# arun-sub/genomicsbench

Measured on AMD Instinct MI355X. Metric: bsw_large_gcups, higher is better.
Workload: dtype int32

## Files before the change

### genomicsbench_amd/csrc/bsw_kernels.hip

```cpp
#include "gbx_internal.h"
#include <atomic>
#include <cstdlib>

namespace gbx {
namespace {

constexpr int NEG = -(1 << 29);
constexpr int BIGJ = 1 << 20;

constexpr int NCLS = 21;
constexpr int CLS_LDS = NCLS - 1;
constexpr int NTB = 32;
constexpr int NBIN = NCLS * NTB;
constexpr int HDR = 1024;
constexpr int REG_SCORE_LIMIT = 1 << 20;

struct BswDev {
    int o_del, e_del, o_ins, e_ins, oe_del, oe_ins, zdrop, end_bonus, w, max_mat;
    uint32_t colword[5];
    int32_t col4[5];
    uint32_t row0[5];
    uint32_t row1[5];
    uint8_t remap[24];
    uint32_t lrow[5];
// ... 534 lines not shown
            "v_lshl_or_b32 %[wn], %[v], 16, %[u]\n"
            : [sa] "=&v"(sa), [ta] "=&v"(ta), [tb] "=&v"(tb), [ma] "=&v"(ma), [mb] "=&v"(mb), [x] "=&v"(x), [ha] "=&v"(ha),
              [hb] "=&v"(hb), [td] "=&v"(td), [ed] "=&v"(ed), [ena] "=&v"(ena), [enb] "=&v"(enb), [fd] "=&v"(fd), [ka] "=&v"(ka),
              [kb] "=&v"(kb), [u] "=&v"(u), [v] "=&v"(v), [wn] "=&v"(wn), [f] "+v"(f), [key] "=v"(kout)
            : [w] "v"(w), [qq] "v"(qq), [rw] "v"(rw), [rwn] "v"(rwn), [left] "v"(left), [kin] "v"(kin), [pa] "v"(pa), [pa1] "v"(pa1), [zero] "v"(zero), [oed] "s"(oe_del),
              [edel] "s"(e_del), [eins] "s"(e_ins)
            : "vcc");
    } else {
        int sa, ta, tb, ma, mb, x, ha, td, ti, ed, ena, enb, fd, ka, kb, u, v;
        asm volatile(
            "v_perm_b32 %[sa], %[rwn], %[rw], %[qq]\n"
            "v_cmp_ne_u32_sdwa vcc, %[w], %[zero] src0_sel:BYTE_1 src1_sel:DWORD\n"
            "v_subrev_u32 %[fd], %[eins], %[f]\n"
            "v_add_u32_sdwa %[ta], sext(%[sa]), %[w] dst_sel:DWORD dst_unused:UNUSED_PAD src0_sel:BYTE_0 src1_sel:BYTE_1\n"
            "v_cndmask_b32 %[ma], 0, %[ta], vcc\n"
            "v_cmp_ne_u32_sdwa vcc, %[w], %[zero] src0_sel:BYTE_3 src1_sel:DWORD\n"
            "v_max_i32_sdwa %[x], %[ma], %[w] dst_sel:DWORD dst_unused:UNUSED_PAD src0_sel:DWORD src1_sel:BYTE_0\n"
            "v_add_u32_sdwa %[tb], sext(%[sa]), %[w] dst_sel:DWORD dst_unused:UNUSED_PAD src0_sel:BYTE_1 src1_sel:BYTE_3\n"
            "v_max_i32 %[ha], %[x], %[f]\n"
            "v_subrev_u32 %[td], %[oed], %[ma]\n"
            "v_subrev_u32 %[ti], %[oei], %[ma]\n"
            "v_cndmask_b32 %[mb], 0, %[tb], vcc\n"
            "v_sub_u32_sdwa %[ed], %[w], %[edel] dst_sel:DWORD dst_unused:UNUSED_PAD src0_sel:BYTE_0 src1_sel:DWORD\n"
            "v_max3_i32 %[f], %[fd], %[ti], 0\n"
            "v_max3_i32 %[ena], %[ed], %[td], 0\n"
            "v_max_i32_sdwa %[x], %[mb], %[w] dst_sel:DWORD dst_unused:UNUSED_PAD src0_sel:DWORD src1_sel:BYTE_2\n"
            "v_lshl_or_b32 %[ka], %[ha], 18, %[pa]\n"
            "v_max_i32 %[hb], %[x], %[f]\n"
            "v_subrev_u32 %[td], %[oed], %[mb]\n"
            "v_subrev_u32 %[ti], %[oei], %[mb]\n"
            "v_subrev_u32 %[fd], %[eins], %[f]\n"
            "v_sub_u32_sdwa %[ed], %[w], %[edel] dst_sel:DWORD dst_unused:UNUSED_PAD src0_sel:BYTE_2 src1_sel:DWORD\n"
            "v_max3_i32 %[f], %[fd], %[ti], 0\n"
            "v_max3_i32 %[enb], %[ed], %[td], 0\n"
            "v_lshl_or_b32 %[kb], %[hb], 18, %[pa1]\n"
            "v_lshl_or_b32 %[u], %[left], 8, %[ena]\n"
            "v_lshl_or_b32 %[v], %[ha], 8, %[enb]\n"
            "v_max3_u32 %[key], %[kin], %[ka], %[kb]\n"
            "v_lshl_or_b32 %[wn], %[v], 16, %[u]\n"
            : [sa] "=&v"(sa), [ta] "=&v"(ta), [tb] "=&v"(tb), [ma] "=&v"(ma), [mb] "=&v"(mb), [x] "=&v"(x), [ha] "=&v"(ha),
              [hb] "=&v"(hb), [td] "=&v"(td), [ti] "=&v"(ti), [ed] "=&v"(ed), [ena] "=&v"(ena), [enb] "=&v"(enb), [fd] "=&v"(fd), [ka] "=&v"(ka),
              [kb] "=&v"(kb), [u] "=&v"(u), [v] "=&v"(v), [wn] "=&v"(wn), [f] "+v"(f), [key] "=v"(kout)
            : [w] "v"(w), [qq] "v"(qq), [rw] "v"(rw), [rwn] "v"(rwn), [left] "v"(left), [kin] "v"(kin), [pa] "v"(pa), [pa1] "v"(pa1), [zero] "v"(zero), [oed] "s"(oe_del),
              [oei] "s"(oe_ins), [edel] "s"(e_del), [eins] "s"(e_ins)
            : "vcc");
    }
    left = hb;
    key = kout;
    return wn;
}

#ifdef GBX_BSW_LANE_STATS
__device__ unsigned long long g_bsw_lane_stats[16][4];
#endif
template <bool SYM, bool COMPACT, bool CODE4 = false, bool PACKED = false>
__global__ void __launch_bounds__(64) bsw_lane_kernel(BswDev prm, BswPairs P, BswWork W, int rlo, int rhi, int cols, int slot)
{
    extern __shared__ uint32_t lcell[];
#ifdef GBX_BSW_LANE_STATS
    __shared__ int st_rowmax[2048];
    for (int k = threadIdx.x; k < 2048; k += 64) st_rowmax[k] = 0;
    unsigned long long st_cells = 0, st_rows = 0, st_wcells = 0, st_wrows = 0;
#endif
#define LCELL(byte_addr) (*(uint32_t *)((char *)lcell + (byte_addr)))
#define LCELL16(byte_addr) (*(uint16_t *)((char *)lcell + (byte_addr)))
#define LQ8(byte_addr) (*((uint8_t *)lcell + (byte_addr)))
    const int lane = threadIdx.x;
    const int first = W.lbase[rlo << 8], count = W.lbase[(rhi + 1) << 8] - first;
    const int nchunks = (count + 63) >> 6;
    const int32_t *order = W.lorder + first;
    const int e_ins = prm.e_ins, e_del = prm.e_del, oe_ins = prm.oe_ins, oe_del = prm.oe_del;
    const int cb = lane * 4;
    constexpr int QROW = CODE4 ? 64 : 128;
    const int qb = (cols >> 1) * 256 + (CODE4 ? lane : (lane & 31) * 4 + (lane >> 5) * 2);
    auto LQREAD = [&](int a) -> uint32_t { return CODE4 ? (uint32_t)LQ8(a) : (uint32_t)LCELL16(a); };
    auto QSEL = [](uint32_t q) -> uint32_t { return CODE4 ? (((q >> 4) << 8) | (q & 15u)) : q; };
    auto QLOW = [](uint32_t q) -> uint32_t { return CODE4 ? (q & 15u) : (q & 0xffu); };
    auto cell_at = [&](int j) { return COMPACT ? (j >> 1) * 256 + cb + (j & 1) * 2 : j * 256 + cb; };
    const int tab = COMPACT ? (cols >> 1) * (256 + QROW) + 512 : (cols + 2) * 256 - 128;
    if (lane < 5) *(uint4 *)((char *)lcell + tab + lane * 16) = make_uint4(prm.row0[lane], prm.row1[lane], prm.lrow[lane], 0u);
#define LTAB(base_code) (*(const uint4 *)((const char *)lcell + tab + min((int)(base_code), 4) * 16))
    int rel0 = 0, rel1 = 2, rel2 = 256, rel3 = 258, rel4 = 512, rel5 = 514, rel6 = 768, rel7 = 770;
    asm volatile("" : "+v"(rel0), "+v"(rel1), "+v"(rel2), "+v"(rel3), "+v"(rel4), "+v"(rel5), "+v"(rel6), "+v"(rel7));
    for (;;) {
        int c = 0;
        if (lane == 0) c = atomicAdd(&W.lchunk[slot], 1);
        c = __builtin_amdgcn_readfirstlane(c);
        if (c >= nchunks) break;
        const int hi_ = count - (c << 6), idx = hi_ - 64 + lane;
        const bool have = idx >= 0;
        const int pair = order[have ? idx : 0];
        const int qlen = P.len2[pair], tlen = P.len1[pair], h0 = P.h0[pair];
        const int64_t qo = P.idq[pair], to = P.idr[pair];
        const uint8_t *q = P.qer + (PACKED ? 0 : qo);
        const uint8_t *t = P.ref + (PACKED ? 0 : to);
        auto qpiece = [&](int j) -> uint4 {
            uint4 r;
            if (!PACKED) { __builtin_memcpy(&r, q + j, 16); return r; }
            const int64_t o = qo + j;
            const uint8_t *b = q + (o >> 1);
            uint64_t v;
            __builtin_memcpy(&v, b, 8);
            if (o & 1) v = (v >> 4) | ((uint64_t)b[8] << 60);
            auto spread = [](unsigned h) -> unsigned { return (h & 0xfu) | ((h & 0xf0u) << 4) | ((h & 0xf00u) << 8) | ((h & 0xf000u) << 12); };
            const unsigned lo = (unsigned)v, hi = (unsigned)(v >> 32);
            r.x = spread(lo & 0xffffu); r.y = spread(lo >> 16); r.z = spread(hi & 0xffffu); r.w = spread(hi >> 16);
            return r;
        };
        auto tbase = [&](int i) -> int {
            if (!PACKED) return t[i];
            const int64_t o = to + i;
            return (t[o >> 1] >> ((int)(o & 1) * 4)) & 15;
        };
        {
            uint4 wq = qpiece(0);
            int hrun = h0 - oe_ins + e_ins;
            for (int j0 = 0; j0 <= qlen; j0 += 16) {
                const uint4 cur = wq;
                if (j0 + 16 <= qlen) wq = qpiece(j0 + 16);
                const uint32_t ww[4] = {cur.x, cur.y, cur.z, cur.w};
#pragma unroll
                for (int c = 0; c < 16; c += 2) {
                    const int j = j0 + c;
                    if (j <= qlen) {
                        const uint32_t two = (ww[c >> 2] >> ((c & 3) * 8)) & 0xffffu;
                        const int c0 = j < qlen ? min((int)(two & 0xffu), 4) : 0, c1 = j + 1 < qlen ? min((int)(two >> 8), 4) : 0;
                        const int hv0 = j == 0 ? h0 : max(hrun, 0), hv1 = max(hrun - e_ins, 0);
                        hrun -= 2 * e_ins;
                        if (COMPACT) {
                            LCELL((j >> 1) * 256 + cb) = ((uint32_t)hv0 << 8) | ((uint32_t)hv1 << 24);
                            if (CODE4) LQ8(qb + (j >> 1) * QROW) = (uint8_t)(c0 | (c1 << 4));
                            else LCELL16(qb + (j >> 1) * QROW) = (uint16_t)(c0 | (c1 << 8));
                        } else {
                            LCELL(cell_at(j)) = ((uint32_t)hv0 << 18) | (uint32_t)(c0 * 6);
                            if (j + 1 <= qlen) LCELL(cell_at(j + 1)) = ((uint32_t)hv1 << 18) | (uint32_t)(c1 * 6);
                        }
                    }
                }
            }
        }
        const int w = band_width(prm, qlen);
        int best = h0, best_i = -1, best_j = -1, g_i = -1, g_score = -1, off = 0;
        int beg = 0, end = qlen;
        uint4 mrow = LTAB(tbase(0)), mnext = LTAB(tbase(1));
        int tb2 = tbase(2);
        const uint8_t *tp = t + 3;
        int hrow = h0 - prm.o_del - e_del;
        int imw = -w, ipw = w + 1;
        for (int i = 0; i < tlen; ++i) {
            const uint32_t rw = COMPACT ? mrow.x : mrow.z, rwn = mrow.y;
            mrow = mnext;
            mnext = LTAB(tb2);
            if (PACKED) tb2 = tbase(i + 3);
            else tb2 = *tp++;
            beg = max(beg, imw);
            end = min(min(end, ipw), qlen);
            ++imw; ++ipw;
#ifdef GBX_BSW_LANE_STATS
            if (have) { st_cells += (unsigned)max(end - beg, 0); st_rows += 1; atomicMax(&st_rowmax[i & 2047], max(end - beg, 0) + 1); }
#endif
            int left = beg == 0 ? max(hrow, 0) : 0;
            hrow -= e_del;
            int f = 0;
            uint32_t key = 0;
            int vzero = 0;
            asm volatile("" : "+v"(vzero));
            uint32_t sb0 = 0, sb1 = 0, se0 = 0, se1 = 0;
            const int sp0 = beg >> 1, sq = max((end >> 1) - 1, 0);
            if (COMPACT) {
                auto step = [&](int diag, int e, uint32_t qc, int at) -> uint32_t {
                    const int sc = (int)(int8_t)__builtin_amdgcn_perm(rwn, rw, qc);
                    const int m = diag ? diag + sc : 0;
                    const int h = imax3(m, e, f);
                    key = max(key, ((uint32_t)h << 18) | (uint32_t)at);
                    const int td = m - oe_del;
                    const int en = imax3(e - e_del, td, 0);
                    f = imax3(f - e_ins, SYM ? td : m - oe_ins, 0);
                    const uint32_t cell = ((uint32_t)left << 8) | (uint32_t)en;
                    left = h;
                    return cell;
                };
                const bool odd_first = (beg & 1) && beg < end;
                int j = odd_first ? beg - 1 : beg;
                int pa = (j >> 1) * 256 + cb, qa = qb + (j >> 1) * QROW;
                uint32_t w0 = LCELL(pa), q0 = LQREAD(qa), w1 = LCELL(pa + 256), q1 = LQREAD(qa + QROW);
                w0 &= odd_first ? 0xffff0000u : 0xffffffffu;
                for (; j + 7 < end; j += 8, pa += 1024, qa += 4 * QROW) {
                    const uint32_t x0 = LCELL(pa + 512), y0 = LQREAD(qa + 2 * QROW), x1 = LCELL(pa + 768), y1 = LQREAD(qa + 3 * QROW);
                    uint32_t kt;
                    LCELL(pa) = lane_pair_step<SYM>(w0, QSEL(q0), rw, rwn, f, left, (uint32_t)vzero, kt, rel0, rel1, vzero, oe_del, oe_ins, e_del, e_ins);
                    LCELL(pa + 256) = lane_pair_step<SYM>(w1, QSEL(q1), rw, rwn, f, left, kt, kt, rel2, rel3, vzero, oe_del, oe_ins, e_del, e_ins);
                    w0 = LCELL(pa + 1024); q0 = LQREAD(qa + 4 * QROW); w1 = LCELL(pa + 1280); q1 = LQREAD(qa + 5 * QROW);
                    LCELL(pa + 512) = lane_pair_step<SYM>(x0, QSEL(y0), rw, rwn, f, left, kt, kt, rel4, rel5, vzero, oe_del, oe_ins, e_del, e_ins);
                    LCELL(pa + 768) = lane_pair_step<SYM>(x1, QSEL(y1), rw, rwn, f, left, kt, kt, rel6, rel7, vzero, oe_del, oe_ins, e_del, e_ins);
                    key = max(key, kt + (uint32_t)pa);
                }
                if (j + 3 < end) {
                    const uint32_t x0 = LCELL(pa + 512), y0 = LQREAD(qa + 2 * QROW);
                    LCELL(pa) = lane_pair_step<SYM>(w0, QSEL(q0), rw, rwn, f, left, key, key, pa, pa + 2, vzero, oe_del, oe_ins, e_del, e_ins);
                    LCELL(pa + 256) = lane_pair_step<SYM>(w1, QSEL(q1), rw, rwn, f, left, key, key, pa + 256, pa + 258, vzero, oe_del, oe_ins, e_del, e_ins);
                    w0 = x0; q0 = y0;
                    w1 = LCELL(pa + 768); q1 = LQREAD(qa + 3 * QROW);
                    j += 4; pa += 512; qa += 2 * QROW;
                }
                if (j + 1 < end) {
                    LCELL(pa) = lane_pair_step<SYM>(w0, QSEL(q0), rw, rwn, f, left, key, key, pa, pa + 2, vzero, oe_del, oe_ins, e_del, e_ins);
                    w0 = w1; q0 = q1;
                    j += 2; pa += 256; qa += QROW;
                }
                if (j < end) {
                    LCELL16(pa) = (uint16_t)step((int)((w0 >> 8) & 0xffu), (int)(w0 & 0xffu), QLOW(q0), pa);
                }
                LCELL16(cell_at(end)) = (uint16_t)(left << 8);
                sb0 = LCELL(sp0 * 256 + cb); sb1 = LCELL(sp0 * 256 + 256 + cb);
                se0 = LCELL(sq * 256 + cb); se1 = LCELL(sq * 256 + 256 + cb);
            } else {
                uint32_t left18 = (uint32_t)left << 18;
                int ab = cell_at(beg);
                const int abend = cell_at(end);
                uint32_t cw = LCELL(ab);
#pragma unroll 2
                for (; ab < abend; ab += 256) {
                    const uint32_t nw = LCELL(ab + 256);
                    const int diag = (int)(cw >> 18), e = (int)((cw >> 5) & 0x1fffu);
                    const uint32_t qo = cw & 31u;
                    const int sc = __builtin_amdgcn_sbfe((int)rw, qo, 6u);
                    const int m = diag ? diag + sc : 0;
                    const int h = imax3(m, e, f);
                    const uint32_t h18 = (uint32_t)h << 18;
                    key = max(key, h18 | (uint32_t)ab);
                    const int td = m - oe_del;
                    const int en = imax3(e - e_del, td, 0);
                    f = imax3(f - e_ins, SYM ? td : m - oe_ins, 0);
                    LCELL(ab) = left18 | ((uint32_t)en << 5) | qo;
                    left18 = h18;
                    cw = nw;
                }
                left = (int)(left18 >> 18);
                LCELL(abend) = left18 | (LCELL(abend) & 31u);
            }
            const int jfin = beg < end ? end : beg;
            if (jfin == qlen) {
                if (!(g_score > left)) g_i = i;
                g_score = max(g_score, left);
            }
            const int row_best = (int)(key >> 18);
            const int karg = (int)(key & 0x3ffffu) - cb;
            const int row_arg = COMPACT ? ((karg >> 8) << 1) | ((karg >> 1) & 1) : karg >> 8;
            if (row_best == 0) break;
            if (row_best > best) {
                best = row_best; best_i = i; best_j = row_arg;
                off = max(off, abs(row_arg - i));
            } else if (prm.zdrop > 0) {
                const int di = i - best_i, dj = row_arg - best_j;
                if (di > dj) { if (best - row_best - (di - dj) * e_del > prm.zdrop) break; }
                else if (best - row_best - (dj - di) * e_ins > prm.zdrop) break;
            }
            int j = beg;
            if (COMPACT) {
                int k = (sb1 >> 16) ? 3 : 4;
                k = (sb1 & 0xffffu) ? 2 : k;
                k = (sb0 >> 16) ? 1 : k;
                k = (sb0 & 0xffffu) && !(beg & 1) ? 0 : k;
                j = 2 * sp0 + k;
                if (k == 4) while (j < end && LCELL16(cell_at(j)) == 0) ++j;
                j = min(j, end);
                const int nbeg = beg < end ? j : beg;
                const int khi = end - 2 * sq;
                k = (se0 & 0xffffu) ? 0 : -1;
                k = (se0 >> 16) && khi >= 1 ? 1 : k;
                k = (se1 & 0xffffu) && khi >= 2 ? 2 : k;
                k = (se1 >> 16) && khi >= 3 ? 3 : k;
                j = 2 * sq + k;
                if (k < 0 && 2 * sq > nbeg) while (j >= nbeg && LCELL16(cell_at(j)) == 0) --j;
                j = max(j, nbeg - 1);
                j = nbeg > end ? end : j;
                beg = nbeg;
            } else {
                while (j < end && LCELL(cell_at(j)) < 32u) ++j;
                beg = j;
                j = end;
                while (j >= beg && LCELL(cell_at(j)) < 32u) --j;
            }
            end = min(j + 2, qlen);
        }
        gbx_bsw_result r;
        r.score = best; r.tle = best_i + 1; r.gtle = g_i + 1; r.qle = best_j + 1; r.gscore = g_score; r.max_off = off;
        if (have) P.out[pair] = r;
#ifdef GBX_BSW_LANE_STATS
        __builtin_amdgcn_s_waitcnt(0);
        for (int k = threadIdx.x; k < 2048; k += 64) { const int m = st_rowmax[k]; if (m) { st_wcells += 64ull * (unsigned)(m - 1); st_wrows += 64; } st_rowmax[k] = 0; }
#endif
    }
#ifdef GBX_BSW_LANE_STATS
    atomicAdd(&g_bsw_lane_stats[slot][0], st_cells); atomicAdd(&g_bsw_lane_stats[slot][1], st_wcells);
    atomicAdd(&g_bsw_lane_stats[slot][2], st_rows); atomicAdd(&g_bsw_lane_stats[slot][3], st_wrows);
#endif
#undef LCELL
#undef LCELL16
#undef LQ8
#undef LTAB
}

struct RowShape { int lpp, cpl; };
typedef void (*RowsFn)(BswDev, BswPairs, BswWork, int);
struct RowKernel { int lpp, cpl; RowsFn fn[2]; std::atomic<int> bpc[2]; const char *name; };
#define GBX_ROW_KERNEL(L, C) { L, C, { bsw_rows_kernel<L, C, false>, bsw_rows_kernel<L, C, true> }, { 0, 0 }, "bsw_rows_" #L "x" #C }
RowKernel row_kernels[] = {
    GBX_ROW_KERNEL(2, 4),  GBX_ROW_KERNEL(2, 8),  GBX_ROW_KERNEL(2, 12), GBX_ROW_KERNEL(2, 16), GBX_ROW_KERNEL(2, 20), GBX_ROW_KERNEL(2, 24),
    GBX_ROW_KERNEL(4, 14), GBX_ROW_KERNEL(4, 16), GBX_ROW_KERNEL(4, 18), GBX_ROW_KERNEL(4, 20), GBX_ROW_KERNEL(4, 22), GBX_ROW_KERNEL(4, 24),
    GBX_ROW_KERNEL(8, 13), GBX_ROW_KERNEL(8, 14), GBX_ROW_KERNEL(8, 15), GBX_ROW_KERNEL(8, 16),
    GBX_ROW_KERNEL(16, 10), GBX_ROW_KERNEL(16, 12), GBX_ROW_KERNEL(16, 16), GBX_ROW_KERNEL(64, 16),
    GBX_ROW_KERNEL(4, 8), GBX_ROW_KERNEL(4, 12), GBX_ROW_KERNEL(8, 10), GBX_ROW_KERNEL(8, 12), GBX_ROW_KERNEL(16, 8),
    GBX_ROW_KERNEL(64, 3), GBX_ROW_KERNEL(64, 4),
};
#undef GBX_ROW_KERNEL
constexpr int class_qmax[NCLS - 1] = {8, 16, 24, 32, 40, 48, 56, 64, 72, 80, 88, 96, 104, 112, 120, 128, 160, 192, 256, 1024};

constexpr uint8_t CLASS_REMAP[3][NCLS] = {
    {0, 1, 2, 3, 4, 5, 6, 7, 8, 9, 10, 11, 12, 13, 14, 15, 16, 17, 18, 19, 20},
    {3, 3, 3, 3, 7, 7, 7, 7, 11, 11, 11, 11, 15, 15, 15, 15, 18, 18, 18, 19, 20},
    {15, 15, 15, 15, 15, 15, 15, 15, 15, 15, 15, 15, 15, 15, 15, 15, 18, 18, 18, 19, 20},
};
int class_mode_for(int64_t n)
{
    const char *e = getenv("GBX_BSW_CLASSMODE");
    if (e && *e >= '0' && *e <= '2') return *e - '0';
    return n < 32768 ? 2 : n < 250000 ? 1 : 0;
}

RowKernel *find_row_kernel(int lpp, int cpl)
{
    for (RowKernel &k : row_kernels)
        if (k.lpp == lpp && k.cpl == cpl) return &k;
    return nullptr;
}

const RowShape *class_shapes()
{
    static RowShape shapes[NCLS - 1] = {{2, 4},  {2, 8},  {2, 12}, {2, 16}, {2, 20}, {2, 24}, {4, 14}, {4, 16}, {4, 18}, {4, 20},
                                        {4, 22}, {4, 24}, {8, 13}, {8, 14}, {8, 15}, {8, 16}, {16, 10}, {16, 12}, {16, 16}, {64, 16}};
    static bool parsed = false;
    if (!parsed) {
        parsed = true;
        const char *e = getenv("GBX_BSW_SHAPES");
        for (int c = 0; e && *e && c < NCLS - 1; ++c) {
            int l = 0, k = 0, used = 0;
            if (sscanf(e, "%dx%d%n", &l, &k, &used) != 2) break;
            if (find_row_kernel(l, k) && l * k >= class_qmax[c]) shapes[c] = {l, k};
            e += used;
            if (*e == ',') ++e;
        }
    }
    return shapes;
}

int make_dev_params(const gbx_bsw_params *p, BswDev *d)
{
    if (p->e_del < 1 || p->e_ins < 1 || p->o_del < 0 || p->o_ins < 0 || p->e_del > 4096 || p->e_ins > 4096 ||
        p->o_del > (1 << 16) || p->o_ins > (1 << 16) || p->w < 0) {
        set_error("bsw: gap penalties must satisfy 0<=o<=65536, 1<=e<=4096, w>=0");
        return GBX_ERR_ARG;
    }
    d->o_del = p->o_del; d->e_del = p->e_del; d->o_ins = p->o_ins; d->e_ins = p->e_ins;
    d->oe_del = p->o_del + p->e_del; d->oe_ins = p->o_ins + p->e_ins;
    d->zdrop = p->zdrop; d->end_bonus = p->end_bonus; d->w = p->w;
    int mx = 0;
    for (int k = 0; k < 25; ++k) mx = p->mat[k] > mx ? p->mat[k] : mx;
    d->max_mat = mx;
    for (int q = 0; q < 5; ++q) {
        uint32_t wv = 0;
        for (int t = 0; t < 4; ++t) wv |= (uint32_t)(uint8_t)p->mat[t * 5 + q] << (8 * t);
        d->colword[q] = wv;
        d->col4[q] = p->mat[4 * 5 + q];
    }
    for (int t = 0; t < 5; ++t) {
        uint32_t wv = 0;
        for (int q = 0; q < 4; ++q) wv |= (uint32_t)(uint8_t)p->mat[t * 5 + q] << (8 * q);
        d->row0[t] = wv;
        d->row1[t] = (uint32_t)(uint8_t)p->mat[t * 5 + 4];
    }
    d->lane_on = 0;
    bool fits6 = true;
    for (int k = 0; k < 25; ++k) fits6 = fits6 && p->mat[k] >= -32 && p->mat[k] <= 31;
    for (int t = 0; t < 5; ++t) {
        uint32_t wv = 0;
        for (int q = 0; q < 5; ++q) wv |= ((uint32_t)p->mat[t * 5 + q] & 63u) << (6 * q);
        d->lrow[t] = wv;
    }
    if (fits6 && p->o_del + p->e_del < LANE_SCORE_LIMIT && p->o_ins + p->e_ins < LANE_SCORE_LIMIT) d->lane_on = -1;
    return GBX_OK;
}

}

constexpr int64_t WS_LANE = (int64_t)(LANE_BINS + 64) + 64;
size_t bsw_workspace_bytes(int64_t n)
{
    return (size_t)(WS_HDR + 4 * (n > 0 ? n : 0) + WS_LANE) * sizeof(int32_t);
}

constexpr int UNPACK_ROUNDS = 4;
__global__ void __launch_bounds__(256) bsw_unpack4_kernel(const uint8_t *__restrict__ packed, uint8_t *__restrict__ out, int64_t lo, int64_t hi)
{
    const int64_t base = lo + (int64_t)blockIdx.x * (256 * 16 * UNPACK_ROUNDS) + threadIdx.x * 16;
    const bool aligned = (((uintptr_t)(packed + (base >> 1)) & 7) == 0) && (((uintptr_t)(out + base) & 15) == 0);
    if (aligned && base + (int64_t)(UNPACK_ROUNDS - 1) * 4096 + 16 <= hi) {
        uint2 v[UNPACK_ROUNDS];
#pragma unroll
        for (int r = 0; r < UNPACK_ROUNDS; ++r) v[r] = *(const uint2 *)(packed + ((base + r * 4096) >> 1));
        auto spread = [](unsigned h) -> unsigned { return (h & 0xfu) | ((h & 0xf0u) << 4) | ((h & 0xf00u) << 8) | ((h & 0xf000u) << 12); };
#pragma unroll
        for (int r = 0; r < UNPACK_ROUNDS; ++r) {
            uint4 q;
            q.x = spread(v[r].x & 0xffffu); q.y = spread(v[r].x >> 16); q.z = spread(v[r].y & 0xffffu); q.w = spread(v[r].y >> 16);
            *(uint4 *)(out + base + r * 4096) = q;
        }
        return;
    }
    for (int r = 0; r < UNPACK_ROUNDS; ++r) {
        const int64_t o = base + r * 4096;
        if (o >= hi) return;
        if (aligned && o + 16 <= hi) {
            const uint2 v = *(const uint2 *)(packed + (o >> 1));
            auto spread = [](unsigned h) -> unsigned { return (h & 0xfu) | ((h & 0xf0u) << 4) | ((h & 0xf00u) << 8) | ((h & 0xf000u) << 12); };
            uint4 q;
            q.x = spread(v.x & 0xffffu); q.y = spread(v.x >> 16); q.z = spread(v.y & 0xffffu); q.w = spread(v.y >> 16);
            *(uint4 *)(out + o) = q;
        } else {
            for (int64_t k = o; k < o + 16 && k < hi; ++k) out[k] = (uint8_t)((packed[k >> 1] >> ((k & 1) * 4)) & 0xf);
        }
    }
}

int bsw_unpack4(const uint8_t *d_packed, uint8_t *d_out, int64_t lo, int64_t hi, hipStream_t s)
{
    if (hi <= lo) return GBX_OK;
    const int64_t per_block = 256 * 16 * UNPACK_ROUNDS;
    Stage st("bsw_unpack4", s);
    hipLaunchKernelGGL(bsw_unpack4_kernel, dim3((unsigned)((hi - lo + per_block - 1) / per_block)), dim3(256), 0, s, d_packed, d_out, lo, hi);
    GBX_HIP(hipGetLastError());
    return GBX_OK;
}

int bsw_launch_direct(const gbx_bsw_params *p, int64_t n, int max_qlen,
                      const uint8_t *d_ref, const uint8_t *d_qer, const int64_t *d_idr, const int64_t *d_idq,
                      const int32_t *d_len1, const int32_t *d_len2, const int32_t *d_h0, gbx_bsw_result *d_out, hipStream_t s)
{
    if (n <= 0) return GBX_OK;
    BswDev dev;
    int rc = make_dev_params(p, &dev);
    if (rc) return rc;
    for (int c = 0; c < NCLS; ++c) dev.remap[c] = (uint8_t)c;
    BswPairs P = {d_ref, d_qer, d_idr, d_idq, d_len1, d_len2, d_h0, d_out};
    BswWork W = {nullptr, nullptr, nullptr, nullptr, nullptr, nullptr, nullptr, nullptr, nullptr, nullptr};
    dev.lane_on = 0;
    if (max_qlen > 256) { set_error("bsw: direct launch needs queries of at most 256"); return GBX_ERR_ARG; }
    const int cols = max_qlen + 1;
    int lpp = 16, cpl = cols <= 128 ? 8 : cols <= 160 ? 10 : cols <= 192 ? 12 : 16;
    if (n < 4096) { lpp = 64; cpl = cols <= 192 ? 3 : 4; }
    if (const char *e = getenv("GBX_BSW_DIRECT_SHAPE")) {
        int l = 0, c = 0;
        if (sscanf(e, "%dx%d", &l, &c) == 2 && l * c > max_qlen && find_row_kernel(l, c)) { lpp = l; cpl = c; }
    }
    RowKernel *k = find_row_kernel(lpp, cpl);
    if (!k) { set_error("bsw: no %dx%d row kernel", lpp, cpl); return GBX_ERR_UNSUPPORTED; }
    const bool sym = dev.oe_ins == dev.oe_del;
    const int gpb = 256 / lpp;
    const int blocks = (int)((n + gpb - 1) / gpb);
    Stage st(k->name, s);
    hipLaunchKernelGGL(k->fn[sym], dim3(blocks), dim3(256), 0, s, dev, P, W, -(int)n);
    GBX_HIP(hipGetLastError());
    return GBX_OK;
}

static bool lane_wanted(int64_t n)
{
    const char *lane_env = getenv("GBX_BSW_LANE");
    const int64_t lane_min = getenv("GBX_BSW_LANE_MIN") ? atoll(getenv("GBX_BSW_LANE_MIN")) : 262144;
    return lane_env ? atoi(lane_env) != 0 : n >= lane_min;
}

int bsw_lane_rule(const gbx_bsw_params *p, int64_t n, BswLaneRule *r)
{
    BswDev dev;
    const int rc = make_dev_params(p, &dev);
    if (rc) return rc;
    r->on = dev.lane_on && lane_wanted(n) ? 1 : 0;
    r->max_mat = dev.max_mat > 0 ? dev.max_mat : 0;
    r->qmax = LANE_QMAX;
    r->limit = LANE_SCORE_LIMIT;
    r->compact_limit = LANE_COMPACT_LIMIT;
    static_assert(LANE_NRANGE == 5, "BswLaneRule::range_hi / BswChunkPrep::class_pairs");
    for (int f = 0; f < 2; ++f) for (int k = 0; k < LANE_NRANGE; ++k) r->range_hi[f][k] = LANE_RANGE_HI[f][k];
    return GBX_OK;
}

int bsw_launch(const gbx_bsw_params *p, int64_t n,
               const uint8_t *d_ref, const uint8_t *d_qer,
               const int64_t *d_idr, const int64_t *d_idq,
               const int32_t *d_len1, const int32_t *d_len2, const int32_t *d_h0,
               gbx_bsw_result *d_out, void *d_work, size_t work_bytes, hipStream_t s, hipEvent_t *join_events,
               const BswChunkPrep *prep)
{
    if (n == 0) return GBX_OK;
    if (n > 0x7fffffffLL - 1024) { set_error("bsw: more than 2^31 pairs in one call"); return GBX_ERR_UNSUPPORTED; }
    if (work_bytes < bsw_workspace_bytes(n)) { set_error("bsw: workspace too small"); return GBX_ERR_ARG; }
    BswDev dev;
    int rc = make_dev_params(p, &dev);
    if (rc) return rc;
    const int mode = class_mode_for(n);
    for (int c = 0; c < NCLS; ++c) dev.remap[c] = CLASS_REMAP[mode][c];
    BswPairs P = {d_ref, d_qer, d_idr, d_idq, d_len1, d_len2, d_h0, d_out};
    int32_t *wi = (int32_t *)d_work;
    int32_t *wl = wi + WS_HDR + 4 * n;
    BswWork W = {wi, wi + HDR, wi + 2 * HDR, wi + 3 * HDR, wi + WS_HDR, wi + WS_HDR + n, wl, wi + WS_HDR + 3 * n, wi + WS_HDR + 2 * n,
                 wl + LANE_BINS + 64};
    dev.lane_on = dev.lane_on && lane_wanted(n) ? 1 : 0;
    static const bool serial = getenv("GBX_BSW_SERIAL") != nullptr;
    SideStreams *ss = nullptr;
    std::unique_lock<std::mutex> side_lock;
    if (!serial) {
        if ((rc = side_streams(&ss))) return rc;
        side_lock = std::unique_lock<std::mutex>(ss->mu);
    }
    static const bool prep_off = getenv("GBX_BSW_PREP") && atoi(getenv("GBX_BSW_PREP")) == 0;
    const bool ahead = prep && prep->uploaded && join_events && !serial && !prep_off;
    hipStream_t s_cls = ahead ? ss->pre[0] : s;
    const bool no_rows = dev.lane_on && prep && prep->rows_pairs == 0 && !(getenv("GBX_BSW_SKIP_ROWS") && atoi(getenv("GBX_BSW_SKIP_ROWS")) == 0);
    const bool packed_lanes = no_rows && prep->ref_packed && !(getenv("GBX_BSW_PACKED_LANES") && atoi(getenv("GBX_BSW_PACKED_LANES")) == 0);
    const int phase = prep ? prep->phase : 0;
    if (phase && !(ahead && packed_lanes && prep->ev_pre && prep->ev_aux)) {
        if (phase == 1) return 1;
        set_error("bsw: the kernels of a chunk whose preparing passes were not queued");
        return GBX_ERR_ARG;
    }
    hipEvent_t ev_pre = phase ? prep->ev_pre : ss ? ss->ev_pre : nullptr, ev_aux = phase ? prep->ev_aux : ss ? ss->ev_aux : nullptr;
    const bool sort_aside = dev.lane_on && !serial;
    if (packed_lanes) { P.ref = prep->ref_packed; P.qer = prep->qer_packed; P.packed = 1; }
    if (phase != 2) {
        if (ahead) {
            GBX_HIP(hipStreamWaitEvent(ss->pre[0], prep->uploaded, 0));
            GBX_HIP(hipStreamWaitEvent(ss->pre[1], prep->uploaded, 0));
        }
        if (!packed_lanes && prep && prep->ref_packed) {
            const int64_t from_r = prep->unp_r ? *prep->unp_r : prep->lo_r, from_q = prep->unp_q ? *prep->unp_q : prep->lo_q;
            if ((rc = bsw_unpack4(prep->ref_packed, prep->ref_bytes, from_r, prep->hi_r, s_cls)) ||
                (rc = bsw_unpack4(prep->qer_packed, prep->qer_bytes, from_q, prep->hi_q, s_cls)))
                return rc;
            if (prep->unp_r && prep->hi_r > *prep->unp_r) *prep->unp_r = prep->hi_r;
            if (prep->unp_q && prep->hi_q > *prep->unp_q) *prep->unp_q = prep->hi_q;
        }
        GBX_HIP(hipMemsetAsync(d_work, 0, WS_HDR * sizeof(int32_t), s_cls));
        if (dev.lane_on) {
            hipStream_t so = s;
            if (ahead) {
                so = ss->pre[1];
                GBX_HIP(hipMemsetAsync(wl, 0, (size_t)WS_LANE * sizeof(int32_t), so));
            } else {
                GBX_HIP(hipMemsetAsync(wl, 0, (size_t)WS_LANE * sizeof(int32_t), s));
                if (sort_aside) {
                    if ((rc = ss->fork(s))) return rc;
                    so = ss->side[SideStreams::N - 1];
                }
            }
            Stage st("bsw_lane_sort", so);
            const int sblocks = (int)((n + 255) / 256);
            hipLaunchKernelGGL(bsw_lane_sort_kernel, dim3(sblocks), dim3(256), 0, so, dev, P, n, W, 0);
            hipLaunchKernelGGL(bsw_lane_scan_kernel, dim3(1), dim3(1024), 0, so, W);
            hipLaunchKernelGGL(bsw_lane_sort_kernel, dim3(sblocks), dim3(256), 0, so, dev, P, n, W, 1);
            if (sort_aside) GBX_HIP(hipEventRecord(ev_aux, so));
        }
        const int cblocks = (int)((n + CLS_THREADS - 1) / CLS_THREADS);
        {
            Stage st("bsw_classify", s_cls);
            hipLaunchKernelGGL(bsw_classify_kernel, dim3(cblocks), dim3(CLS_THREADS), 0, s_cls, dev, P, n, W, 0);
            hipLaunchKernelGGL(bsw_scan_kernel, dim3(1), dim3(HDR), 0, s_cls, W);
            hipLaunchKernelGGL(bsw_classify_kernel, dim3(cblocks), dim3(CLS_THREADS), 0, s_cls, dev, P, n, W, 1);
        }
        if (ahead) GBX_HIP(hipEventRecord(ev_pre, s_cls));
        GBX_HIP(hipGetLastError());
        if (phase == 1) return GBX_OK;
    }
    if (ahead) {
        GBX_HIP(hipStreamWaitEvent(s, ev_pre, 0));
        for (int k = 0; k < SideStreams::N; ++k) GBX_HIP(hipStreamWaitEvent(ss->side[k], ev_pre, 0));
        if (phase == 2) {
            GBX_HIP(hipStreamWaitEvent(s, prep->uploaded, 0));
            for (int k = 0; k < SideStreams::N; ++k) GBX_HIP(hipStreamWaitEvent(ss->side[k], prep->uploaded, 0));
        }
    }

    int dev_id = 0, cus = 256;
    (void)hipGetDevice(&dev_id);
    (void)hipDeviceGetAttribute(&cus, hipDeviceAttributeMultiprocessorCount, dev_id);
    auto grid_for = [&](int groups_per_block, int blocks_per_cu) {
        int64_t want = (n + groups_per_block - 1) / groups_per_block;
        int64_t cap = (int64_t)cus * blocks_per_cu;
        return (int)(want < cap ? want : cap);
    };
    const bool sym = dev.oe_ins == dev.oe_del;
    const RowShape *shapes = class_shapes();
    if (!serial && !sort_aside && !ahead && (rc = ss->fork(s))) return rc;
    int launched = 0;
    for (int c = 0; c < NCLS - 1 && !no_rows; ++c) {
        if (CLASS_REMAP[mode][c] != c) continue;
        static const int nk_env = getenv("GBX_BSW_KSTREAMS") ? atoi(getenv("GBX_BSW_KSTREAMS")) : 0;
        const int nk = nk_env > 0 ? nk_env : join_events ? 3 : 4;
        const int lane_k = mode ? launched++ % (nk > 4 ? 4 : nk) : nk >= 4 ? (c & 3) : c % nk;
        hipStream_t sc = serial || sort_aside || lane_k == 0 ? s : ss->side[lane_k - 1];
        RowKernel *k = find_row_kernel(shapes[c].lpp, shapes[c].cpl);
        if (!k) { set_error("bsw: no row kernel for class %d", c); return GBX_ERR_UNSUPPORTED; }
        int bpc = k->bpc[sym].load(std::memory_order_relaxed);
        if (!bpc) {
            int q = 0;
            if (hipOccupancyMaxActiveBlocksPerMultiprocessor(&q, k->fn[sym], 256, 0) != hipSuccess || q < 1) {
                (void)hipGetLastError();
                q = 2;
            }
            bpc = q > 8 ? 8 : q;
            k->bpc[sym].store(bpc, std::memory_order_relaxed);
        }
        Stage st(k->name, sc);
        hipLaunchKernelGGL(k->fn[sym], dim3(grid_for(256 / k->lpp, bpc)), dim3(256), 0, sc, dev, P, W, c);
    }
    if (sort_aside) {
        GBX_HIP(hipStreamWaitEvent(s, ev_aux, 0));
        for (int k = 0; k + (ahead ? 0 : 1) < SideStreams::N; ++k) GBX_HIP(hipStreamWaitEvent(ss->side[k], ev_aux, 0));
    }
    if (dev.lane_on) {
        static const char *names[2][LANE_NRANGE] = {{"bsw_lane_c47", "bsw_lane_c79", "bsw_lane_c99", "bsw_lane_c135", "bsw_lane_c159"},
                                                    {"bsw_lane_w39", "bsw_lane_w79", "bsw_lane_w103", "bsw_lane_w127", "bsw_lane_w159"}};
        for (int fmt = 1; fmt >= 0; --fmt) {
            int nl = 0;
            for (int r = LANE_NRANGE - 1; r >= 0; --r) {
                const int qlo = r ? LANE_RANGE_HI[fmt][r - 1] + 1 : 1, qhi = LANE_RANGE_HI[fmt][r];
                static const bool skip_on = getenv("GBX_BSW_SKIP_EMPTY") && atoi(getenv("GBX_BSW_SKIP_EMPTY")) == 1;
                if (skip_on && prep && prep->class_known && prep->class_pairs[fmt * LANE_NRANGE + r] == 0) continue;
                ++nl;
                const int cols = (qhi + 3) & ~1;
                const char *c4e = getenv("GBX_BSW_CODE4");
                const bool code4 = fmt == 0 && (c4e ? atoi(c4e) != 0 : qhi > 99);
                const size_t lds = fmt ? (size_t)(cols + 2) * 256 : (size_t)(cols / 2) * (code4 ? 320 : 384) + 640;
                int per_cu = (int)((size_t)160 * 1024 / lds);
                if (per_cu > 16) per_cu = 16;
                const int sk = (nl - 1) & 3;
                hipStream_t sc = serial || sk == 0 ? s : ss->side[sk - 1];
                int64_t blocks = (int64_t)cus * per_cu, want = (n + 63) / 64;
                if (blocks > want) blocks = want;
                const int rlo = fmt * (LANE_QMAX + 1) + qlo, rhi = fmt * (LANE_QMAX + 1) + qhi, slot = fmt * LANE_NRANGE + r;
                Stage st(names[fmt][r], sc);
                auto go = [&](auto kern) { hipLaunchKernelGGL(kern, dim3((unsigned)blocks), dim3(64), lds, sc, dev, P, W, rlo, rhi, cols, slot); };
                if (P.packed) {
                    if (fmt == 0 && code4) { if (sym) go(bsw_lane_kernel<true, true, true, true>); else go(bsw_lane_kernel<false, true, true, true>); }
                    else if (fmt == 0) { if (sym) go(bsw_lane_kernel<true, true, false, true>); else go(bsw_lane_kernel<false, true, false, true>); }
                    else { if (sym) go(bsw_lane_kernel<true, false, false, true>); else go(bsw_lane_kernel<false, false, false, true>); }
                } else if (fmt == 0 && code4) {
                    if (sym) go(bsw_lane_kernel<true, true, true>); else go(bsw_lane_kernel<false, true, true>);
                } else if (fmt == 0) {
                    if (sym) go(bsw_lane_kernel<true, true>); else go(bsw_lane_kernel<false, true>);
                } else {
                    if (sym) go(bsw_lane_kernel<true, false>); else go(bsw_lane_kernel<false, false>);
                }
            }
        }
    }
    if (!serial && !join_events && (rc = ss->join(s))) return rc;
    if (!no_rows) {
        const size_t lds_bytes = (size_t)(GBX_BSW_MAX_QLEN + 1) * 2 * sizeof(int);
        static std::atomic<uint64_t> attr_set[2];
        int cur = 0;
        GBX_HIP(hipGetDevice(&cur));
        const uint64_t bit = (uint64_t)1 << (cur & 63);
        if (cur >= 128 || !(attr_set[cur >> 6].load(std::memory_order_acquire) & bit)) {
            GBX_HIP(hipFuncSetAttribute((const void *)bsw_lds_kernel, hipFuncAttributeMaxDynamicSharedMemorySize, (int)lds_bytes));
            if (cur < 128) attr_set[cur >> 6].fetch_or(bit, std::memory_order_release);
        }
        int blocks = (int)(n < (int64_t)cus * 2 ? n : (int64_t)cus * 2);
        Stage st("bsw_lds", s);
        hipLaunchKernelGGL(bsw_lds_kernel, dim3(blocks), dim3(64), lds_bytes, s, dev, P, W, CLS_LDS);
    }
    if (join_events) {
        if (!ss && (rc = side_streams(&ss))) return rc;
        GBX_HIP(hipEventRecord(join_events[0], s));
        for (int k = 0; k < SideStreams::N; ++k) GBX_HIP(hipEventRecord(join_events[1 + k], ss->side[k]));
    }
    GBX_HIP(hipGetLastError());
    return GBX_OK;
}

}

#ifdef GBX_BSW_LANE_STATS
extern "C" int gbx_debug_bsw_lane_stats(unsigned long long *out, int reset)
{
    if (hipMemcpyFromSymbol(out, HIP_SYMBOL(gbx::g_bsw_lane_stats), sizeof(unsigned long long) * 64) != hipSuccess) return -1;
    if (reset) { unsigned long long z[64] = {0}; if (hipMemcpyToSymbol(HIP_SYMBOL(gbx::g_bsw_lane_stats), z, sizeof(z)) != hipSuccess) return -1; }
    return 0;
}
#endif
```

Before: 2435.

## Add register-resident lane kernel with inline-asm cell step for mid-length queries

New measurement: 2524 (median of 6 runs). 3.6% higher.

```diff
diff --git a/genomicsbench_amd/csrc/bsw_kernels.hip b/genomicsbench_amd/csrc/bsw_kernels.hip
--- a/genomicsbench_amd/csrc/bsw_kernels.hip
+++ b/genomicsbench_amd/csrc/bsw_kernels.hip
@@ -860,6 +860,328 @@
 #undef LTAB
 }
 
+
+#define GBX_REG_STEP_HEAD(SEL0, SEL1)                                                                                                   \
+    "v_cmp_ne_u32_sdwa vcc, %[w], %[zero] src0_sel:BYTE_1 src1_sel:DWORD\n"                                                            \
+    "v_subrev_u32 %[fd], %[eins], %[f]\n"                                                                                               \
+    "v_add_u32_sdwa %[ta], sext(%[sa]), %[w] dst_sel:DWORD dst_unused:UNUSED_PAD src0_sel:" SEL0 " src1_sel:BYTE_1\n"                  \
+    "v_cndmask_b32 %[ma], 0, %[ta], vcc\n"                                                                                              \
+    "v_cmp_ne_u32_sdwa vcc, %[w], %[zero] src0_sel:BYTE_3 src1_sel:DWORD\n"                                                            \
+    "v_max_i32_sdwa %[x], %[ma], %[w] dst_sel:DWORD dst_unused:UNUSED_PAD src0_sel:DWORD src1_sel:BYTE_0\n"                            \
+    "v_add_u32_sdwa %[tb], sext(%[sa]), %[w] dst_sel:DWORD dst_unused:UNUSED_PAD src0_sel:" SEL1 " src1_sel:BYTE_3\n"                  \
+    "v_max_i32 %[ha], %[x], %[f]\n"
+#define GBX_REG_STEP_SYM(SEL0, SEL1)                                                                                                    \
+    GBX_REG_STEP_HEAD(SEL0, SEL1)                                                                                                       \
+    "v_subrev_u32 %[td], %[oed], %[ma]\n"                                                                                               \
+    "v_cndmask_b32 %[mb], 0, %[tb], vcc\n"                                                                                              \
+    "v_sub_u32_sdwa %[ed], %[w], %[edel] dst_sel:DWORD dst_unused:UNUSED_PAD src0_sel:BYTE_0 src1_sel:DWORD\n"                         \
+    "v_max3_i32 %[f], %[fd], %[td], 0\n"                                                                                                \
+    "v_max3_i32 %[ena], %[ed], %[td], 0\n"                                                                                              \
+    "v_max_i32_sdwa %[x], %[mb], %[w] dst_sel:DWORD dst_unused:UNUSED_PAD src0_sel:DWORD src1_sel:BYTE_2\n"                            \
+    "v_lshl_or_b32 %[ka], %[ha], 18, %[pa]\n"                                                                                           \
+    "v_max_i32 %[hb], %[x], %[f]\n"                                                                                                     \
+    "v_subrev_u32 %[td], %[oed], %[mb]\n"                                                                                               \
+    "v_subrev_u32 %[fd], %[eins], %[f]\n"                                                                                               \
+    "v_sub_u32_sdwa %[ed], %[w], %[edel] dst_sel:DWORD dst_unused:UNUSED_PAD src0_sel:BYTE_2 src1_sel:DWORD\n"                         \
+    "v_max3_i32 %[f], %[fd], %[td], 0\n"                                                                                                \
+    "v_max3_i32 %[enb], %[ed], %[td], 0\n"                                                                                              \
+    "v_lshl_or_b32 %[kb], %[hb], 18, %[pa1]\n"                                                                                          \
+    "v_lshl_or_b32 %[u], %[left], 8, %[ena]\n"                                                                                          \
+    "v_lshl_or_b32 %[v], %[ha], 8, %[enb]\n"                                                                                            \
+    "v_max3_u32 %[key], %[kin], %[ka], %[kb]\n"                                                                                         \
+    "v_lshl_or_b32 %[wn], %[v], 16, %[u]\n"
+#define GBX_REG_STEP_ASYM(SEL0, SEL1)                                                                                                   \
+    GBX_REG_STEP_HEAD(SEL0, SEL1)                                                                                                       \
+    "v_subrev_u32 %[td], %[oed], %[ma]\n"                                                                                               \
+    "v_subrev_u32 %[ti], %[oei], %[ma]\n"                                                                                               \
+    "v_cndmask_b32 %[mb], 0, %[tb], vcc\n"                                                                                              \
+    "v_sub_u32_sdwa %[ed], %[w], %[edel] dst_sel:DWORD dst_unused:UNUSED_PAD src0_sel:BYTE_0 src1_sel:DWORD\n"                         \
+    "v_max3_i32 %[f], %[fd], %[ti], 0\n"                                                                                                \
+    "v_max3_i32 %[ena], %[ed], %[td], 0\n"                                                                                              \
+    "v_max_i32_sdwa %[x], %[mb], %[w] dst_sel:DWORD dst_unused:UNUSED_PAD src0_sel:DWORD src1_sel:BYTE_2\n"                            \
+    "v_lshl_or_b32 %[ka], %[ha], 18, %[pa]\n"                                                                                           \
+    "v_max_i32 %[hb], %[x], %[f]\n"                                                                                                     \
+    "v_subrev_u32 %[td], %[oed], %[mb]\n"                                                                                               \
+    "v_subrev_u32 %[ti], %[oei], %[mb]\n"                                                                                               \
+    "v_subrev_u32 %[fd], %[eins], %[f]\n"                                                                                               \
+    "v_sub_u32_sdwa %[ed], %[w], %[edel] dst_sel:DWORD dst_unused:UNUSED_PAD src0_sel:BYTE_2 src1_sel:DWORD\n"                         \
+    "v_max3_i32 %[f], %[fd], %[ti], 0\n"                                                                                                \
+    "v_max3_i32 %[enb], %[ed], %[td], 0\n"                                                                                              \
+    "v_lshl_or_b32 %[kb], %[hb], 18, %[pa1]\n"                                                                                          \
+    "v_lshl_or_b32 %[u], %[left], 8, %[ena]\n"                                                                                          \
+    "v_lshl_or_b32 %[v], %[ha], 8, %[enb]\n"                                                                                            \
+    "v_max3_u32 %[key], %[kin], %[ka], %[kb]\n"                                                                                         \
+    "v_lshl_or_b32 %[wn], %[v], 16, %[u]\n"
+template <bool SYM, bool HI, int PA>
+__device__ __forceinline__ uint32_t reg_pair_step(uint32_t w, uint32_t sa, int &f, int &left, uint32_t &key, int zero, int oe_del, int oe_ins,
+                                                  int e_del, int e_ins)
+{
+    uint32_t wn, kout;
+    int hb, ta, tb, ma, mb, x, ha, td, ti, ed, ena, enb, fd, ka, kb, u, v;
+#define GBX_REG_STEP_OPS                                                                                                                \
+    : [ta] "=&v"(ta), [tb] "=&v"(tb), [ma] "=&v"(ma), [mb] "=&v"(mb), [x] "=&v"(x), [ha] "=&v"(ha), [hb] "=&v"(hb), [td] "=&v"(td),   \
+      [ti] "=&v"(ti), [ed] "=&v"(ed), [ena] "=&v"(ena), [enb] "=&v"(enb), [fd] "=&v"(fd), [ka] "=&v"(ka), [kb] "=&v"(kb), [u] "=&v"(u), \
+      [v] "=&v"(v), [wn] "=&v"(wn), [f] "+v"(f), [key] "=v"(kout)                                                                       \
+    : [w] "v"(w), [sa] "v"(sa), [left] "v"(left), [kin] "v"(key), [pa] "i"(PA), [pa1] "i"(PA + 1), [zero] "v"(zero), [oed] "s"(oe_del), \
+      [oei] "s"(oe_ins), [edel] "s"(e_del), [eins] "s"(e_ins)                                                                           \
+    : "vcc"
+    if (SYM && !HI) asm volatile(GBX_REG_STEP_SYM("BYTE_0", "BYTE_1") GBX_REG_STEP_OPS);
+    if (SYM && HI) asm volatile(GBX_REG_STEP_SYM("BYTE_2", "BYTE_3") GBX_REG_STEP_OPS);
+    if (!SYM && !HI) asm volatile(GBX_REG_STEP_ASYM("BYTE_0", "BYTE_1") GBX_REG_STEP_OPS);
+    if (!SYM && HI) asm volatile(GBX_REG_STEP_ASYM("BYTE_2", "BYTE_3") GBX_REG_STEP_OPS);
+#undef GBX_REG_STEP_OPS
+    (void)ti;
+    left = hb;
+    key = kout;
+    return wn;
+}
+#undef GBX_REG_STEP_SYM
+#undef GBX_REG_STEP_ASYM
+#undef GBX_REG_STEP_HEAD
+
+template <bool AND>
+__device__ inline uint32_t wave_bits(uint32_t x)
+{
+    auto op = [](uint32_t a, uint32_t b) { return AND ? a & b : a | b; };
+    int y = (int)x;
+    y = (int)op(y, dpp<0x111>(y, y));
+    y = (int)op(y, dpp<0x112>(y, y));
+    y = (int)op(y, dpp<0x114>(y, y));
+    y = (int)op(y, dpp<0x118>(y, y));
+    y = (int)op(y, dpp<0x142, 0xa>(y, y));
+    y = (int)op(y, dpp<0x143, 0xc>(y, y));
+    return (uint32_t)__builtin_amdgcn_readlane(y, 63);
+}
+__device__ inline uint32_t bits_from(int lo)
+{
+    return lo <= 0 ? ~0u : lo >= 32 ? 0u : ~0u << lo;
+}
+__device__ inline uint32_t bit_span(int lo, int hi)
+{
+    return lo > hi ? 0u : (hi >= 31 ? ~0u : (2u << hi) - 1u) & ~((1u << lo) - 1u);
+}
+
+template <bool SYM, bool HI, int PA>
+__device__ __forceinline__ void reg_pair_masked(uint32_t &cell, uint32_t sa, int beg, int end, int &f, int &left, uint32_t &key,
+                                                int zero, int oe_del, int oe_ins, int e_del, int e_ins)
+{
+    constexpr int c0 = PA;
+    if (c0 + 1 < end && c0 + 1 >= beg) {
+        const uint32_t win = c0 < beg ? cell & 0xffff0000u : cell;
+        cell = reg_pair_step<SYM, HI, PA>(win, sa, f, left, key, zero, oe_del, oe_ins, e_del, e_ins);
+    } else if (c0 + 1 == end) {
+        if (c0 >= beg) {
+            const int sc = (int)(int8_t)(sa >> (HI ? 16 : 0));
+            const int diag = (int)((cell >> 8) & 0xffu), e = (int)(cell & 0xffu);
+            const int m = diag ? diag + sc : 0;
+            const int h = imax3(m, e, f);
+            key = max(key, ((uint32_t)h << 18) | (uint32_t)PA);
+            const int en = imax3(e - e_del, m - oe_del, 0);
+            cell = ((uint32_t)h << 24) | ((uint32_t)left << 8) | (uint32_t)en;
+            left = h;
+        } else {
+            cell = (cell & 0xffffu) | ((uint32_t)left << 24);
+        }
+    } else if (c0 == end) {
+        cell = (cell & 0xffff0000u) | ((uint32_t)left << 8);
+    }
+}
+
+template <bool SYM, int QHI>
+__global__ void __launch_bounds__(64, 3) bsw_lane_reg_kernel(BswDev prm, BswPairs P, BswWork W, int rlo, int rhi, int slot)
+{
+    constexpr int NCP = QHI / 2 + 1;
+    constexpr int NB = (NCP + 3) / 4;
+    constexpr int NQ = (NCP + 1) / 2;
+    constexpr int NW = (2 * NCP + 31) / 32;
+    static_assert(NB <= 31, "block masks are 32-bit");
+    constexpr int OUT = 1 << 12;
+    __shared__ uint2 s_tab[5];
+    const int lane = threadIdx.x;
+    if (lane < 5) s_tab[lane] = make_uint2(prm.row0[lane], prm.row1[lane]);
+    __syncthreads();
+    const int first = W.lbase[rlo << 8], count = W.lbase[(rhi + 1) << 8] - first;
+    const int nchunks = (count + 63) >> 6;
+    const int32_t *order = W.lorder + first;
+    const int e_ins = prm.e_ins, e_del = prm.e_del, oe_ins = prm.oe_ins, oe_del = prm.oe_del;
+    for (;;) {
+        int c = 0;
+        if (lane == 0) c = atomicAdd(&W.lchunk[slot], 1);
+        c = __builtin_amdgcn_readfirstlane(c);
+        if (c >= nchunks) break;
+        const int hi_ = count - (c << 6), idx = hi_ - 64 + lane;
+        const bool have = idx >= 0;
+        const int pair = order[have ? idx : 0];
+        const int qlen = P.len2[pair], tlen = P.len1[pair], h0 = P.h0[pair];
+        const uint8_t *q = P.qer + P.idq[pair];
+        const uint8_t *t = P.ref + P.idr[pair];
+
+        uint32_t qs[NQ];
+#pragma unroll
+        for (int k = 0; k < (4 * NQ + 15) / 16; ++k) {
+            uint4 v = make_uint4(0u, 0u, 0u, 0u);
+            if (16 * k <= qlen) __builtin_memcpy(&v, q + 16 * k, 16);
+            const uint32_t vv[4] = {v.x, v.y, v.z, v.w};
+#pragma unroll
+            for (int m = 0; m < 4 && 4 * k + m < NQ; ++m) {
+                const uint32_t x = vv[m];
+                const uint32_t ge5 = ((((x | 0x80808080u) - 0x05050505u) | x) & 0x80808080u) >> 7;
+                const uint32_t msk = ge5 * 0xffu;
+                qs[4 * k + m] = (x & ~msk) | (0x04040404u & msk);
+            }
+        }
+        uint32_t cell[NCP];
+        {
+            int hr = h0 - oe_ins, rem = qlen;
+#pragma unroll
+            for (int p = 0; p < NCP; ++p) {
+                const int hv0 = p == 0 ? h0 : max(hr + e_ins, 0), hv1 = max(hr, 0);
+                cell[p] = (rem >= 0 ? (uint32_t)hv0 << 8 : 0u) | (rem >= 1 ? (uint32_t)hv1 << 24 : 0u);
+                hr -= 2 * e_ins;
+                rem -= 2;
+            }
+        }
+        const int w = band_width(prm, qlen);
+        int best = h0, best_i = -1, best_j = -1, g_i = -1, g_score = -1, off = 0;
+        int beg = 0, end = qlen;
+        bool running = true;
+        uint2 mrow = s_tab[min((int)t[0], 4)], mnext = s_tab[min((int)t[1], 4)];
+        int tb2 = t[2];
+        const uint8_t *tp = t + 3;
+        int hrow = h0 - prm.o_del - e_del;
+        int imw = -w, ipw = w + 1;
+        for (int i = 0;; ++i) {
+            if (!__any(running)) break;
+            const uint32_t rw = mrow.x, rwn = mrow.y;
+            mrow = mnext;
+            mnext = s_tab[min(tb2, 4)];
+            tb2 = running ? (int)*tp : 0;
+            tp += running ? 1 : 0;
+            beg = max(beg, imw);
+            end = min(min(end, ipw), qlen);
+            ++imw; ++ipw;
+            int left = beg == 0 ? max(hrow, 0) : 0;
+            hrow -= e_del;
+            const int bb = running ? beg : OUT, ee = running ? end : OUT;
+            const int sp0 = bb >> 1, sq = max((ee >> 1) - 1, 0);
+            const uint32_t touch = running ? bit_span(bb >> 3, min(ee >> 3, NB - 1)) : 0u;
+            const uint32_t whole = running ? bit_span((bb + 7) >> 3, min((ee >> 3) - 1, NB - 1)) : ~0u;
+            auto blk = [](int pp) { return pp < 4 * NB ? 1u << (pp >> 2) : 0u; };
+            const uint32_t probe = running ? blk(sp0) | blk(sp0 + 1) | blk(sq) | blk(sq + 1) : 0u;
+            const uint32_t touch_w = wave_bits<false>(touch), whole_w = wave_bits<true>(whole), probe_w = wave_bits<false>(probe);
+            int vzero = 0;
+            asm volatile("" : "+v"(vzero));
+            int f = 0;
+            uint32_t key = 0;
+#pragma unroll
+            for (int b = 0; b < NB; ++b) {
+                if (!((touch_w >> b) & 1u)) continue;
+                const uint32_t sa0 = __builtin_amdgcn_perm(rwn, rw, qs[2 * b]);
+                const uint32_t sa1 = 2 * b + 1 < NQ ? __builtin_amdgcn_perm(rwn, rw, qs[2 * b + 1]) : 0u;
+                uint32_t kt = (uint32_t)vzero;
+                if ((whole_w >> b) & 1u) {
+                    cell[4 * b] = reg_pair_step<SYM, false, 0>(cell[4 * b], sa0, f, left, kt, vzero, oe_del, oe_ins, e_del, e_ins);
+                    if (4 * b + 1 < NCP) cell[4 * b + 1] = reg_pair_step<SYM, true, 2>(cell[4 * b + 1], sa0, f, left, kt, vzero, oe_del, oe_ins, e_del, e_ins);
+                    if (4 * b + 2 < NCP) cell[4 * b + 2] = reg_pair_step<SYM, false, 4>(cell[4 * b + 2], sa1, f, left, kt, vzero, oe_del, oe_ins, e_del, e_ins);
+                    if (4 * b + 3 < NCP) cell[4 * b + 3] = reg_pair_step<SYM, true, 6>(cell[4 * b + 3], sa1, f, left, kt, vzero, oe_del, oe_ins, e_del, e_ins);
+                } else {
+                    int lb = bb - 8 * b, le = ee - 8 * b;
+                    asm volatile("" : "+v"(lb), "+v"(le));
+                    reg_pair_masked<SYM, false, 0>(cell[4 * b], sa0, lb, le, f, left, kt, vzero, oe_del, oe_ins, e_del, e_ins);
+                    if (4 * b + 1 < NCP) reg_pair_masked<SYM, true, 2>(cell[4 * b + 1], sa0, lb, le, f, left, kt, vzero, oe_del, oe_ins, e_del, e_ins);
+                    if (4 * b + 2 < NCP) reg_pair_masked<SYM, false, 4>(cell[4 * b + 2], sa1, lb, le, f, left, kt, vzero, oe_del, oe_ins, e_del, e_ins);
+                    if (4 * b + 3 < NCP) reg_pair_masked<SYM, true, 6>(cell[4 * b + 3], sa1, lb, le, f, left, kt, vzero, oe_del, oe_ins, e_del, e_ins);
+                }
+                key = max(key, kt + (uint32_t)(8 * b));
+            }
+            uint32_t sb0 = 0, sb1 = 0, se0 = 0, se1 = 0;
+#pragma unroll
+            for (int b = 0; b < NB; ++b) {
+                if (!((probe_w >> b) & 1u)) continue;
+                int db = sp0 - 4 * b, de = sq - 4 * b;
+                asm volatile("" : "+v"(db), "+v"(de));
+#pragma unroll
+                for (int m = 0; m < 4 && 4 * b + m < NCP; ++m) {
+                    const uint32_t cv = cell[4 * b + m];
+                    sb0 = db == m ? cv : sb0;
+                    sb1 = db == m - 1 ? cv : sb1;
+                    se0 = de == m ? cv : se0;
+                    se1 = de == m - 1 ? cv : se1;
+                }
+            }
+            if (running) {
+                const int jfin = beg < end ? end : beg;
+                if (jfin == qlen) {
+                    if (!(g_score > left)) g_i = i;
+                    g_score = max(g_score, left);
+                }
+                const int row_best = (int)(key >> 18), row_arg = (int)(key & 0x3ffffu);
+                bool stop = row_best == 0;
+                if (!stop) {
+                    if (row_best > best) {
+                        best = row_best; best_i = i; best_j = row_arg;
+                        off = max(off, abs(row_arg - i));
+                    } else if (prm.zdrop > 0) {
+                        const int di = i - best_i, dj = row_arg - best_j;
+                        stop = di > dj ? best - row_best - (di - dj) * e_del > prm.zdrop : best - row_best - (dj - di) * e_ins > prm.zdrop;
+                    }
+                }
+                if (!stop) {
+                    int k = (sb1 >> 16) ? 3 : 4;
+                    k = (sb1 & 0xffffu) ? 2 : k;
+                    k = (sb0 >> 16) ? 1 : k;
+                    k = (sb0 & 0xffffu) && !(beg & 1) ? 0 : k;
+                    int j = 2 * sp0 + k;
+                    const int khi = end - 2 * sq;
+                    int ke = (se0 & 0xffffu) ? 0 : -1;
+                    ke = (se0 >> 16) && khi >= 1 ? 1 : ke;
+                    ke = (se1 & 0xffffu) && khi >= 2 ? 2 : ke;
+                    ke = (se1 >> 16) && khi >= 3 ? 3 : ke;
+                    uint32_t nz[NW];
+                    if (k == 4 || ke < 0) {
+#pragma unroll
+                        for (int u = 0; u < NW; ++u) nz[u] = 0u;
+#pragma unroll
+                        for (int p = 0; p < NCP; ++p) {
+                            const uint32_t two = ((cell[p] & 0xffffu) ? 1u : 0u) | ((cell[p] >> 16) ? 2u : 0u);
+                            nz[p >> 4] |= two << ((2 * p) & 31);
+                        }
+                    }
+                    if (k == 4) {
+                        int jn = end;
+#pragma unroll
+                        for (int u = NW - 1; u >= 0; --u) {
+                            const uint32_t m = nz[u] & bits_from(j - 32 * u) & ~bits_from(end - 32 * u);
+                            jn = m ? 32 * u + __builtin_ctz(m) : jn;
+                        }
+                        j = jn;
+                    }
+                    j = min(j, end);
+                    const int nbeg = beg < end ? j : beg;
+                    j = 2 * sq + ke;
+                    if (ke < 0 && 2 * sq > nbeg) {
+                        int jl = nbeg - 1;
+#pragma unroll
+                        for (int u = 0; u < NW; ++u) {
+                            const uint32_t m = nz[u] & bits_from(nbeg - 32 * u) & ~bits_from(j + 1 - 32 * u);
+                            jl = m ? 32 * u + 31 - __builtin_clz(m) : jl;
+                        }
+                        j = jl;
+                    }
+                    j = max(j, nbeg - 1);
+                    j = nbeg > end ? end : j;
+                    beg = nbeg;
+                    end = min(j + 2, qlen);
+                }
+                running = !stop && i + 1 < tlen;
+            }
+        }
+        gbx_bsw_result r;
+        r.score = best; r.tle = best_i + 1; r.gtle = g_i + 1; r.qle = best_j + 1; r.gscore = g_score; r.max_off = off;
+        if (have) P.out[pair] = r;
+    }
+}
+
 struct RowShape { int lpp, cpl; };
 typedef void (*RowsFn)(BswDev, BswPairs, BswWork, int);
 struct RowKernel { int lpp, cpl; RowsFn fn[2]; std::atomic<int> bpc[2]; const char *name; };
@@ -1031,6 +1353,8 @@
     GBX_HIP(hipGetLastError());
     return GBX_OK;
 }
+
+static std::atomic<long long> g_lane_reg_launches{0};
 
 static bool lane_wanted(int64_t n)
 {
@@ -1208,6 +1532,25 @@
                 if (blocks > want) blocks = want;
                 const int rlo = fmt * (LANE_QMAX + 1) + qlo, rhi = fmt * (LANE_QMAX + 1) + qhi, slot = fmt * LANE_NRANGE + r;
                 Stage st(names[fmt][r], sc);
+                const char *rege = getenv("GBX_BSW_LANE_REG");
+                if (fmt == 0 && !P.packed && qhi == 99 && !(rege && atoi(rege) == 0)) {
+                    static_assert(LANE_RANGE_HI[0][2] == 99, "bsw_lane_reg_kernel instance");
+                    typedef void (*LaneRegFn)(BswDev, BswPairs, BswWork, int, int, int);
+                    static const LaneRegFn reg_fn[2] = {bsw_lane_reg_kernel<false, 99>, bsw_lane_reg_kernel<true, 99>};
+                    static std::atomic<int> reg_bpc[2];
+                    const LaneRegFn fn = reg_fn[sym];
+                    std::atomic<int> &bc = reg_bpc[sym];
+                    int bpc = bc.load(std::memory_order_relaxed);
+                    if (!bpc) {
+                        if (hipOccupancyMaxActiveBlocksPerMultiprocessor(&bpc, (const void *)fn, 64, 0) != hipSuccess || bpc < 1) { (void)hipGetLastError(); bpc = 8; }
+                        bc.store(bpc, std::memory_order_relaxed);
+                    }
+                    int64_t rblocks = (int64_t)cus * bpc;
+                    if (rblocks > want) rblocks = want;
+                    hipLaunchKernelGGL(fn, dim3((unsigned)rblocks), dim3(64), 0, sc, dev, P, W, rlo, rhi, slot);
+                    g_lane_reg_launches.fetch_add(1, std::memory_order_relaxed);
+                    continue;
+                }
                 auto go = [&](auto kern) { hipLaunchKernelGGL(kern, dim3((unsigned)blocks), dim3(64), lds, sc, dev, P, W, rlo, rhi, cols, slot); };
                 if (P.packed) {
                     if (fmt == 0 && code4) { if (sym) go(bsw_lane_kernel<true, true, true, true>); else go(bsw_lane_kernel<false, true, true, true>); }
@@ -1249,6 +1592,11 @@
 
 }
 
+extern "C" long long gbx_debug_bsw_lane_reg_launches(void)
+{
+    return gbx::g_lane_reg_launches.load(std::memory_order_relaxed);
+}
+
 #ifdef GBX_BSW_LANE_STATS
 extern "C" int gbx_debug_bsw_lane_stats(unsigned long long *out, int reset)
 {
```
